# soedinglab/MMseqs2

Hardware: AMD Instinct MI355X
Metric: sw_gcells_per_s (higher is better)
Workload: dtype int16

## Files before the change

mmseqs2_amd/csrc/mmgpu_api.hip:

```cpp
#include <algorithm>
#include <atomic>
#include <thread>
#include <cmath>
#include <cstdio>
#include <cstring>
#include <numeric>
#include <string>
#include <vector>

#include "mmgpu_internal.h"

#include <chrono>

using namespace mmgpu;

namespace mmgpu {
thread_local std::string g_last_error;
}
using mmgpu::g_last_error;

extern "C" const char *mmgpu_last_error(void) { return g_last_error.c_str(); }

extern "C" int mmgpu_init(mmgpu_ctx **out, int device_id) {
    if (!out) return fail(MMGPU_ERR_ARG, "mmgpu_init: ctx is NULL");
// ... 818 lines not shown
        const bool same_list = d > from && Q.target_ids == qs[deferred[d - 1].query].target_ids && Q.n_targets == qs[deferred[d - 1].query].n_targets;
        if (!same_list) {
            ord.resize(Q.n_targets);
            std::iota(ord.begin(), ord.end(), 0u);
            for (uint32_t k = 0; k < Q.n_targets; k++)
                if (Q.target_ids[k] >= tv.n) { P.bad = true; break; }
            if (P.bad) continue;
            std::stable_sort(ord.begin(), ord.end(), [&](uint32_t a, uint32_t bb) {
                return tv.h_len[Q.target_ids[a]] > tv.h_len[Q.target_ids[bb]];
            });
        }
        for (uint32_t k = 0; k < Q.n_targets; k++) {
            const uint32_t t = Q.target_ids[ord[k]];
            hit_target[D.hit_cursor + k] = t;
            hit_out[D.hit_cursor + k] = D.out_cursor + ord[k];
            P.sum_cells += (uint64_t)Q.qlen * tv.h_len[t];
            P.max_tlen = std::max(P.max_tlen, tv.h_len[t]);
        }
        for (uint32_t k = 0; k < Q.n_targets;) {
            uint64_t jc = 0;
            uint32_t e = k;
            while (e < Q.n_targets && e - k < JOB_HITS) {
                const uint32_t stop = std::min<uint32_t>(e + D.round, Q.n_targets);
                for (; e < stop; e++) jc += (uint64_t)Q.qlen * tv.h_len[hit_target[D.hit_cursor + e]];
                const uint32_t held = e - k;
                if (jc >= JOB_CELLS && (held <= 16 || held % JOB_ROUND == 0)) break;
            }
            SwJob j;
            j.query = D.query;
            j.hit_begin = D.hit_cursor + k;
            j.hit_end = D.hit_cursor + e;
            j.shape = D.shape;
            P.jobs.push_back(j);
            P.cells.push_back(jc);
            k = e;
        }
        if (Q.n_targets) P.rev_mid_len = tv.h_len[hit_target[D.hit_cursor + Q.n_targets / 2]];
        if (mode >= MMGPU_SW_START)
            for (uint32_t k = 0; k < Q.n_targets; k++) b->h_out_target[D.out_cursor + k] = Q.target_ids[k];
    }
}

void SwPrepare::cut_list_jobs() {
    per_query.resize(deferred.size());
    static const unsigned host_threads = std::min(16u, std::max(1u, std::thread::hardware_concurrency()));
    const size_t n_thr = std::max<size_t>(1, std::min<size_t>(host_threads, total_hits / 65536 + 1));
    if (n_thr <= 1) {
        cut_list_jobs_of(0, deferred.size());
        return;
    }
    std::vector<std::thread> pool;
    size_t from = 0;
    uint64_t acc = 0;
    const uint64_t share = total_hits / n_thr + 1;
    for (size_t d = 0; d < deferred.size(); d++) {
        acc += qs[deferred[d].query].n_targets;
        if (acc >= share || d + 1 == deferred.size()) {
            pool.emplace_back(&SwPrepare::cut_list_jobs_of, this, from, d + 1);
            from = d + 1;
            acc = 0;
        }
    }
    for (std::thread &t : pool) t.join();
}

int SwPrepare::join_list_jobs() {
    for (size_t d = 0; d < deferred.size(); d++) {
        const Deferred &D = deferred[d];
        PerQuery &P = per_query[d];
        if (P.bad) return fail(MMGPU_ERR_ARG, "mmgpu_sw_prepare: target id out of range");
        b->cells += P.sum_cells;
        max_tlen = std::max(max_tlen, P.max_tlen);
        for (size_t z = 0; z < P.jobs.size(); z++) {
            SwJob j = P.jobs[z];
            if (D.multi) j.shape |= n_multi++ << 8;
            jobs.push_back(j);
            job_cells.push_back(P.cells[z]);
        }
        const uint32_t n_t = qs[D.query].n_targets;
        if (D.multi && mode >= MMGPU_SW_START && n_t)
            add_rev_jobs(D.query, D.hit_cursor, n_t, D.shape, (uint64_t)qs[D.query].qlen * (P.rev_mid_len + 1));
    }
    return MMGPU_OK;
}

void SwPrepare::order_jobs() {
    sorted.resize(jobs.size());
    std::vector<uint32_t> ord(jobs.size());
    std::iota(ord.begin(), ord.end(), 0u);
    std::stable_sort(ord.begin(), ord.end(), [&](uint32_t a, uint32_t bb) {
        const int ga = sw_shape_group(jobs[a].shape & 0xFFu), gb = sw_shape_group(jobs[bb].shape & 0xFFu);
        return ga != gb ? ga < gb : job_cells[a] > job_cells[bb];
    });
    for (size_t z = 0; z < ord.size(); z++) {
        sorted[z] = jobs[ord[z]];
        b->group_begin[sw_shape_group(sorted[z].shape & 0xFFu) + 1]++;
    }
    for (int g = 0; g < SW_GROUPS; g++) b->group_begin[g + 1] += b->group_begin[g];
    b->n_jobs = (uint32_t)sorted.size();
    b->n_multi_jobs = n_multi;
    std::vector<uint32_t> ro(rev_jobs.size());
    std::iota(ro.begin(), ro.end(), 0u);
    std::stable_sort(ro.begin(), ro.end(), [&](uint32_t a, uint32_t bb) { return rev_cells[a] > rev_cells[bb]; });
    for (uint32_t z : ro) sorted.push_back(rev_jobs[z]);
    b->n_rev_jobs = (uint32_t)rev_jobs.size();
}

int SwPrepare::enqueue_uploads() {
    b->pairs = total_hits;
    b->h_qoff = qoff;
    b->from_pf = pf != nullptr;
    b->pf_stride = pf_stride;
    b->slot_stride = pf_stride;
    hipStream_t s = c->stream;
    mat.assign(par->mat, par->mat + par->alphabet * par->alphabet);
    void *pin = nullptr;
    size_t pin_cap = 0, pin_used = 0;
    if (pf) {
        pin_cap = upload_pinned_need(qres.size()) + upload_pinned_need(qcb.size()) + upload_pinned_need(qoff.size() * 4) +
                  upload_pinned_need(qbias.size() * 4) + upload_pinned_need(qminstart.size() * 4) + upload_pinned_need(mat.size()) +
                  upload_pinned_need((jobs.size() + rev_jobs.size()) * sizeof(SwJob)) + upload_pinned_need(qprof.size()) +
                  upload_pinned_need(qprof_off.size() * 4);
        pin = pinned.acquire(c, pin_cap);
    }
    auto up = [&](DevBuf &buf, const auto &vec) { return upload_pinned(buf, vec, s, pin, pin_cap, pin_used); };
    HIP_TRY(up(b->d_qres, qres));
    HIP_TRY(up(b->d_qcb, qcb));
    HIP_TRY(up(b->d_qoff, qoff));
    HIP_TRY(up(b->d_qbias, qbias));
    HIP_TRY(up(b->d_qminstart, qminstart));
    if (b->any_profile) {
        HIP_TRY(up(b->d_qprof, qprof));
        HIP_TRY(up(b->d_qprof_off, qprof_off));
    }
    if (pf) {
        HIP_TRY(b->d_hit_target.alloc(std::max<size_t>((size_t)total_hits, 1) * 4));
        HIP_TRY(b->d_hit_out.alloc(std::max<size_t>((size_t)total_hits, 1) * 4));
        HIP_TRY(b->d_stats.alloc(SW_FROM_PF_STAT_SLOTS * 24));
        HIP_TRY(hipMemsetAsync(b->d_stats.p, 0, SW_FROM_PF_STAT_SLOTS * 24, s));
        HIP_TRY(b->d_pf_counts.alloc(std::max<size_t>(nq, 1) * 4));
        HIP_TRY(b->d_slot_target.alloc(std::max<size_t>((size_t)total_hits, 1) * 4));
    } else {
        HIP_TRY(upload(b->d_hit_target, hit_target, s));
        HIP_TRY(upload(b->d_hit_out, hit_out, s));
    }
    HIP_TRY(up(b->d_mat, mat));
    HIP_TRY(b->d_out.alloc(std::max<size_t>((size_t)total_hits, 1) * sizeof(mmgpu_sw_hit)));
    order_jobs();
    HIP_TRY(up(b->d_jobs, sorted));
    return MMGPU_OK;
}

hipError_t SwPrepare::alloc_scratch(uint32_t longest) {
    b->scratch_cols = longest + 16;
    b->scratch_slots = std::min<uint32_t>(std::max<uint32_t>(std::max<uint32_t>(n_multi, (uint32_t)rev_jobs.size()), 1),
                                          sw_multi_resident_blocks(b->group_lds[SW_GROUPS - 1], mode >= MMGPU_SW_START, c->compute_units));
    hipError_t e = b->d_scratch.alloc((size_t)b->scratch_slots * 4 * 4 * 2 * (size_t)b->scratch_cols * sizeof(uint2));
    if (e != hipSuccess) return e;
    e = b->d_scratch_busy.alloc((size_t)b->scratch_slots * 4);
    if (e != hipSuccess) return e;
    return hipMemsetAsync(b->d_scratch_busy.p, 0, (size_t)b->scratch_slots * 4, c->stream);
}

int SwPrepare::finish_host_lists() {
    if (any_multi) HIP_TRY(alloc_scratch(max_tlen));
    HIP_TRY(hipStreamSynchronize(c->stream));
    return MMGPU_OK;
}

int SwPrepare::order_device_lists() {
    hipStream_t s = c->stream;
    HIP_TRY(hipMemsetAsync(b->d_out.p, 0, std::max<size_t>((size_t)total_hits, 1) * sizeof(mmgpu_sw_hit), s));
    SwFromPfArgs F;
    F.pf_hits = pf->hits;
    F.pf_stride = pf_stride;
    F.hit_count = pf->counts;
    F.stride = pf_stride;
    F.q_off = b->d_qoff.as<uint32_t>();
    F.t_len = tv.len;
    F.hit_target = b->d_hit_target.as<uint32_t>();
    F.hit_out = b->d_hit_out.as<uint32_t>();
    F.cells = b->d_stats.as<unsigned long long>();
    F.pairs = b->d_stats.as<unsigned long long>() + 1;
    F.count_copy = b->d_pf_counts.as<uint32_t>();
    F.slot_target = b->d_slot_target.as<uint32_t>();
    HIP_TRY(launch_sw_from_pf(F, nq, s));
    HIP_TRY(hipStreamSynchronize(s));
    unsigned long long st[3] = {0, 0, 0}, slots[SW_FROM_PF_STAT_SLOTS * 3];
    HIP_TRY(hipMemcpy(slots, b->d_stats.p, sizeof(slots), hipMemcpyDeviceToHost));
    for (int z = 0; z < SW_FROM_PF_STAT_SLOTS; z++) {
        st[0] += slots[z * 3];
        st[1] += slots[z * 3 + 1];
        st[2] = std::max(st[2], slots[z * 3 + 2]);
    }
    b->cells = st[0];
    b->valid_pairs = st[1];
    if (any_multi) {
        HIP_TRY(alloc_scratch((uint32_t)st[2]));
        HIP_TRY(hipStreamSynchronize(s));
    }
    return MMGPU_OK;
}

}

static int sw_prepare_impl(mmgpu_ctx *c, const mmgpu_sw_params *par, const mmgpu_sw_query *qs, uint32_t nq, int mode,
                           const DeviceLists *pf, const mmgpu_sw_masks *masks, mmgpu_sw_batch_t **out) {
    if (!c || !par || !out || (!qs && nq)) return fail(MMGPU_ERR_ARG, "mmgpu_sw_prepare: NULL argument");
    SwPrepare S{c, par, qs, nq, mode, pf, masks};
    if (int e = S.check_params()) return e;
    S.tv = sw_targets(c, nullptr);
    HIP_TRY(hipSetDevice(c->device));
    std::unique_ptr<mmgpu_sw_batch_t, SwBatchFree> b(new mmgpu_sw_batch_t(), SwBatchFree{c});
    S.b = b.get();
    S.new_batch();
    if (int e = S.size_buffers()) return e;
    if (masks)
        if (int e = S.plan_masked()) return e;
    if (int e = S.copy_queries()) return e;
    S.lap("queries copied, buffers sized");
    if (!S.deferred.empty()) {
        S.cut_list_jobs();
        S.lap("lists sorted by target length, jobs cut (threads)");
        if (int e = S.join_list_jobs()) return e;
    }
    S.lap("jobs joined");
    if (int e = S.enqueue_uploads()) return e;
    S.lap("uploads enqueued, jobs ordered");
    if (masks) {
        if (int e = S.gather_masked()) return e;
        S.lap("masked copies of the targets gathered");
    }
    if (int e = pf ? S.order_device_lists() : S.finish_host_lists()) return e;
    S.lap("scratch + stream drained");
    *out = b.release();
    return MMGPU_OK;
}

extern "C" int mmgpu_sw_prepare(mmgpu_ctx *c, const mmgpu_sw_params *par, const mmgpu_sw_query *qs, uint32_t nq,
                                int mode, mmgpu_sw_batch_t **out) {
    return sw_prepare_impl(c, par, qs, nq, mode, nullptr, nullptr, out);
}

extern "C" int mmgpu_sw_prepare_masked(mmgpu_ctx *c, const mmgpu_sw_params *par, const mmgpu_sw_query *qs, uint32_t nq, int mode,
                                       const mmgpu_sw_masks *masks, mmgpu_sw_batch_t **out) {
    if (out) *out = nullptr;
    if (!masks) return fail(MMGPU_ERR_ARG, "mmgpu_sw_prepare_masked: NULL masks");
    return sw_prepare_impl(c, par, qs, nq, mode, nullptr, masks, out);
}

extern "C" int mmgpu_sw_debug_masked_target(mmgpu_ctx *c, mmgpu_sw_batch_t *b, uint32_t pair, uint8_t *out, size_t cap, uint32_t *len) {
    if (!c || !b) return fail(MMGPU_ERR_ARG, "mmgpu_sw_debug_masked_target: NULL argument");
    if (!b->masked) return fail(MMGPU_ERR_STATE, "mmgpu_sw_debug_masked_target: not a batch of mmgpu_sw_prepare_masked");
    if (pair >= b->m_h_len.size()) return fail(MMGPU_ERR_ARG, "mmgpu_sw_debug_masked_target: pair index out of range");
    const uint32_t l = b->m_h_len[pair];
    const size_t bytes = ((size_t)l + 3) & ~(size_t)3;
    if (len) *len = l;
    if (!out && cap == 0) return MMGPU_OK;
    if (cap < bytes || (!out && bytes)) return fail(MMGPU_ERR_ARG, "mmgpu_sw_debug_masked_target: buffer too small (needs (len + 3) & ~3 bytes)");
    HIP_TRY(hipSetDevice(c->device));
    HIP_TRY(hipStreamSynchronize(c->stream));
    uint32_t off4 = 0;
    HIP_TRY(hipMemcpy(&off4, b->m_off4.as<uint32_t>() + pair, 4, hipMemcpyDeviceToHost));
    if (bytes) HIP_TRY(hipMemcpy(out, b->m_res.as<uint8_t>() + (size_t)off4 * 4, bytes, hipMemcpyDeviceToHost));
    return MMGPU_OK;
}

extern "C" int mmgpu_sw_prepare_from_pf(mmgpu_ctx *c, const mmgpu_sw_params *par, const mmgpu_sw_query *qs, uint32_t nq,
                                        int mode, mmgpu_pf_batch_t *pf, mmgpu_sw_batch_t **out) {
    if (!pf) return fail(MMGPU_ERR_ARG, "mmgpu_sw_prepare_from_pf: NULL prefilter batch");
    DeviceLists L;
    uint32_t pf_nq = 0;
    if (!pf_batch_device_lists(pf, &L.hits, &L.counts, &L.stride, &pf_nq))
        return fail(MMGPU_ERR_STATE, "mmgpu_sw_prepare_from_pf: the prefilter batch was never run, or is an exchange batch of a sharded run");
    if (pf_nq != nq) return fail(MMGPU_ERR_ARG, "mmgpu_sw_prepare_from_pf: query count differs from the prefilter batch");
    return sw_prepare_impl(c, par, qs, nq, mode, &L, nullptr, out);
}

extern "C" int mmgpu_sw_prepare_from_lists(mmgpu_ctx *c, const mmgpu_sw_params *par, const mmgpu_sw_query *qs, uint32_t nq, int mode,
                                           const void *d_hits, const void *d_counts, uint32_t stride, mmgpu_sw_batch_t **out) {
    if ((!d_hits || !d_counts) && nq) return fail(MMGPU_ERR_ARG, "mmgpu_sw_prepare_from_lists: NULL list pointers");
    if (stride == 0) return fail(MMGPU_ERR_ARG, "mmgpu_sw_prepare_from_lists: stride must be >= 1");
    DeviceLists L;
    L.hits = (const mmgpu_pf_hit *)d_hits;
    L.counts = (const uint32_t *)d_counts;
    L.stride = stride;
    return sw_prepare_impl(c, par, qs, nq, mode, &L, nullptr, out);
}

extern "C" int mmgpu_sw_prepare_owned(mmgpu_ctx *c, const mmgpu_sw_params *par, const mmgpu_sw_query *qs, uint32_t nq, int mode,
                                      mmgpu_pf_batch_t *merged, mmgpu_sw_batch_t **out) {
    if (!c || !merged || !out) return fail(MMGPU_ERR_ARG, "mmgpu_sw_prepare_owned: NULL argument");
    if (!c->shard.on) return fail(MMGPU_ERR_STATE, "mmgpu_sw_prepare_owned: no shard set (mmgpu_pf_set_shard)");
    const mmgpu_pf_hit *mh = nullptr;
    const uint32_t *mc = nullptr;
    uint32_t stride = 0, mnq = 0;
    if (!mmgpu::pf_batch_merged_lists(merged, &mh, &mc, &stride, &mnq)) return fail(MMGPU_ERR_STATE, "mmgpu_sw_prepare_owned: the prefilter batch holds no merged lists (mmgpu_pf_exchange_merge first)");
    if (mnq != nq) return fail(MMGPU_ERR_ARG, "mmgpu_sw_prepare_owned: query count differs from the prefilter batch");
    HIP_TRY(hipSetDevice(c->device));
    DevBuf lh, lc, ls;
    lh.bind(c->cache); lc.bind(c->cache); ls.bind(c->cache);
    HIP_TRY(lh.alloc(std::max<size_t>((size_t)nq * stride, 1) * sizeof(mmgpu_pf_hit)));
    HIP_TRY(lc.alloc(std::max<size_t>(nq, 1) * 4));
    HIP_TRY(ls.alloc(std::max<size_t>((size_t)nq * stride, 1) * 4));
    PfLocalizeArgs A;
    A.hits = mh;
    A.counts = mc;
// ... 950 lines not shown
```

mmseqs2_amd/csrc/sw_kernel.hip:

```cpp
#include "mmgpu_internal.h"
#include "pf_device.h"

namespace mmgpu {

namespace {

constexpr int GROUP = 16;
constexpr int WAVES = 4;
constexpr int GROUPS_PER_WAVE = 64 / GROUP;
constexpr int HITS_PER_WAVE = 2 * GROUPS_PER_WAVE;
constexpr unsigned NEG2 = 0x80008000u;

typedef short s16x2 __attribute__((ext_vector_type(2)));
typedef unsigned short u16x2 __attribute__((ext_vector_type(2)));

__device__ __forceinline__ unsigned pk_add_sat(unsigned a, unsigned b) {
    return __builtin_bit_cast(unsigned, __builtin_elementwise_add_sat(__builtin_bit_cast(s16x2, a),
                                                                      __builtin_bit_cast(s16x2, b)));
}
__device__ __forceinline__ unsigned pk_max_s(unsigned a, unsigned b) {
    return __builtin_bit_cast(unsigned, __builtin_elementwise_max(__builtin_bit_cast(s16x2, a),
                                                                  __builtin_bit_cast(s16x2, b)));
}
__device__ __forceinline__ unsigned pk_max_u(unsigned a, unsigned b) {
    return __builtin_bit_cast(unsigned, __builtin_elementwise_max(__builtin_bit_cast(u16x2, a),
                                                                  __builtin_bit_cast(u16x2, b)));
}
__device__ __forceinline__ unsigned pk_sub_sat_u(unsigned a, unsigned b) {
    return __builtin_bit_cast(unsigned, __builtin_elementwise_sub_sat(__builtin_bit_cast(u16x2, a),
                                                                      __builtin_bit_cast(u16x2, b)));
}
__device__ __forceinline__ unsigned bfi(unsigned mask, unsigned a, unsigned b) {
    return (a & mask) | (b & ~mask);
}
__device__ __forceinline__ unsigned from_lane_above(unsigned head, unsigned v) {
    return __builtin_amdgcn_update_dpp(head, v, 0x111 , 0xF, 0xF, false);
}

#ifndef MMGPU_SW_PREFETCH
#define MMGPU_SW_PREFETCH 1
#endif
#define SW_KEEP_IN_ROW(x) asm volatile("" : "+v"(x))

template <int R>
struct Tile {
    static constexpr int ROWS = GROUP * R;
    static constexpr int LANE_STRIDE = lane_stride_bytes(R);
    static constexpr int ROW_STRIDE = GROUP * LANE_STRIDE;
};
static_assert(GROUP == 16, "sw_profile_bytes and sw_tiles (mmgpu_internal.h) assume 16-lane groups");

template <int R, bool REV>
__device__ __forceinline__ void build_profile(unsigned char *lds, const uint8_t *q, const int8_t *cb, int qlen,
                                              int tile_base, const int8_t *mat, int alphabet, const int8_t *prof) {
    using T = Tile<R>;
    const int total = (alphabet + 1) * T::ROWS;
    for (int idx = threadIdx.x; idx < total; idx += blockDim.x) {
        const int letter = idx / T::ROWS;
        const int row = idx - letter * T::ROWS;
        const int rg = tile_base + row;
        short v = (short)-32768;
        if (letter < alphabet && rg < qlen) {
            const int qi = REV ? (qlen - 1 - rg) : rg;
            v = prof ? (short)prof[letter * qlen + qi] : (short)((int)mat[letter * alphabet + q[qi]] + (int)cb[qi]);
        }
        const int lane = row / R, r = row - lane * R;
        *reinterpret_cast<short *>(lds + letter * T::ROW_STRIDE + lane * T::LANE_STRIDE + r * 2) = v;
    }
}

__device__ __forceinline__ bool sw_rev_wanted(const SwLaunch &L, uint32_t slot, int min_start) {
    const mmgpu_sw_hit &f = L.out[slot];
    const int s = f.score;
    if (L.rev_mode == 2) return s > 0 && L.rev_force[slot] != 0;
    return s > 0 && s >= min_start && !(L.rev_mode == 1 && f.word != 0);
}

constexpr int SW_REV_JOB_HITS = 1024;
static_assert(SW_REV_JOB_HITS == SW_REV_JOB_MAX, "host and kernel disagree on the reverse job size");
static_assert(SW_LDS_HEADER == SW_REV_JOB_HITS * 2 + 64, "the header holds the live hits and the scheduling words");

template <int R, bool MULTI, bool REV, bool PF>
__device__ __forceinline__ void sw_body(const SwLaunch &L, const SwJob job) {
    using T = Tile<R>;
    extern __shared__ __attribute__((aligned(16))) unsigned char lds_all[];
    uint16_t *live = reinterpret_cast<uint16_t *>(lds_all);
    uint32_t *live_wave = reinterpret_cast<uint32_t *>(lds_all + SW_REV_JOB_HITS * 2);
    uint32_t *next_chunk = reinterpret_cast<uint32_t *>(lds_all + SW_REV_JOB_HITS * 2 + 16);
    unsigned char *lds = lds_all + SW_LDS_HEADER;
    if (MULTI) __builtin_amdgcn_s_setprio(3);
    const int lane = threadIdx.x & 63;
    const int wave = __builtin_amdgcn_readfirstlane(threadIdx.x >> 6);
    const int g = lane & (GROUP - 1);
    const int grp = lane / GROUP;

    const uint32_t qbeg = L.q_off[job.query];
    const int qlen = (int)(L.q_off[job.query + 1] - qbeg);
    const uint8_t *q = L.q_res + qbeg;
    const int8_t *cb = L.q_cb + qbeg;
    const int qbias = L.q_bias[job.query];
    const int8_t *prof = nullptr;
    if (L.q_prof_off) {
        const uint32_t po = L.q_prof_off[job.query];
        if (po != 0xFFFFFFFFu) prof = L.q_prof + po;
    }
    const int n_tiles = MULTI ? (int)sw_tiles((uint32_t)qlen, R) : 1;
    const uint32_t tile_bytes = sw_profile_bytes(R, L.alphabet);
    const bool resident = MULTI && sw_multi_resident((uint32_t)n_tiles, R, L.alphabet, L.resident_lds);
    const bool dynamic = !MULTI || resident;
    auto build_all_tiles = [&]() {
        for (int tile = 0; tile < n_tiles; ++tile)
            build_profile<R, REV>(lds + (uint32_t)tile * tile_bytes, q, cb, qlen, tile * T::ROWS, L.mat, L.alphabet, prof);
        __syncthreads();
    };

    const unsigned go2 = (unsigned)L.gap_open * 0x10001u;
    const unsigned ge2 = (unsigned)L.gap_extend * 0x10001u;
    const unsigned pad_letter = (unsigned)L.alphabet;

    if (threadIdx.x == 0) *next_chunk = 0;
    if (!MULTI && !REV) {
        build_profile<R, REV>(lds, q, cb, qlen, 0, L.mat, L.alphabet, prof);
        __syncthreads();
    }
    if (MULTI && !REV && resident) build_all_tiles();

    uint32_t n_hits = job.hit_end - job.hit_begin;
    if (REV) {
        const int min_start = L.q_minstart[job.query];
        uint32_t total = 0;
        for (uint32_t base = 0; base < n_hits; base += WAVES * 64) {
            const uint32_t idx = base + threadIdx.x;
            bool pass = false;
            if (idx < n_hits) pass = sw_rev_wanted(L, L.hit_out[job.hit_begin + idx], min_start);
            const unsigned long long bal = __ballot(pass);
            if (lane == 0) live_wave[wave] = (uint32_t)__popcll(bal);
            __syncthreads();
            uint32_t before = 0, round_total = 0;
#pragma unroll
            for (int w = 0; w < WAVES; ++w) {
                const uint32_t c = live_wave[w];
                before += w < wave ? c : 0u;
                round_total += c;
            }
            if (pass) live[total + before + (uint32_t)__popcll(bal & ((1ull << lane) - 1ull))] = (uint16_t)idx;
            total += round_total;
            __syncthreads();
        }
        n_hits = total;
        if (n_hits == 0) return;
        if (!MULTI) {
            build_profile<R, REV>(lds, q, cb, qlen, 0, L.mat, L.alphabet, prof);
            __syncthreads();
        }
        if (MULTI && resident) build_all_tiles();
    }
    const uint32_t n_iter = (n_hits + WAVES * HITS_PER_WAVE - 1) / (WAVES * HITS_PER_WAVE);

    for (uint32_t it = 0; dynamic || it < n_iter; ++it) {
        uint32_t chunk = it * WAVES + wave;
        if (dynamic) {
            if (lane == 0) chunk = atomicAdd(next_chunk, 1u);
            chunk = __builtin_amdgcn_readfirstlane(chunk);
        }
        const uint32_t slot0 = chunk * HITS_PER_WAVE;
        if (dynamic && slot0 >= n_hits) break;

        const uint32_t sA = slot0 + grp * 2, sB = sA + 1;
        const bool vA = sA < n_hits, vB = sB < n_hits;
        const uint32_t hA = job.hit_begin + (REV ? (uint32_t)live[vA ? sA : 0] : sA);
        const uint32_t hB = job.hit_begin + (REV ? (uint32_t)live[vB ? sB : 0] : sB);
        const uint32_t tA = vA ? L.hit_target[hA] : 0u, tB = vB ? L.hit_target[hB] : 0u;
        const uint8_t *pA = L.t_res + (size_t)L.t_off4[tA] * 4;
        const uint8_t *pB = L.t_res + (size_t)L.t_off4[tB] * 4;
        int colsA = vA ? (int)L.t_len[tA] : 0, colsB = vB ? (int)L.t_len[tB] : 0;
        int r0A = 0, r0B = 0;
        int endA = 0, endB = 0;
        unsigned rev_target = 0xFFFFFFFFu;
        if (REV) {
            mmgpu_sw_hit fa, fb;
            fa.score = 0; fa.q_end = 0; fa.t_end = 0;
            fb = fa;
            if (vA) fa = L.out[L.hit_out[hA]];
            if (vB) fb = L.out[L.hit_out[hB]];
            colsA = vA ? fa.t_end + 1 : 0;
            colsB = vB ? fb.t_end + 1 : 0;
            endA = colsA > 0 ? fa.t_end : 0;
            endB = colsB > 0 ? fb.t_end : 0;
            r0A = colsA > 0 ? qlen - 1 - fa.q_end : 0;
            r0B = colsB > 0 ? qlen - 1 - fb.q_end : 0;
            rev_target = (colsA > 0 ? (unsigned)fa.score & 0xFFFFu : 0xFFFFu) | ((colsB > 0 ? (unsigned)fb.score & 0xFFFFu : 0xFFFFu) << 16);
        }
        int ncols = colsA > colsB ? colsA : colsB;
        ncols = max(ncols, __shfl_xor(ncols, 16));
        ncols = max(ncols, __shfl_xor(ncols, 32));
        ncols = __builtin_amdgcn_readfirstlane(ncols);
        const int nsteps = ncols + GROUP - 1;

        unsigned long long bestA = 0, bestB = 0;

        uint2 *scr = nullptr;
        if (MULTI) scr = L.scratch + ((size_t)((job.shape >> 8) * WAVES + wave) * GROUPS_PER_WAVE + grp) * 2 * L.scratch_cols;

        for (int tile = 0; tile < n_tiles; ++tile) {
            const int tile_base = tile * T::ROWS;
            if (MULTI && !resident) {
                __syncthreads();
                build_profile<R, REV>(lds, q, cb, qlen, tile_base, L.mat, L.alphabet, prof);
                __syncthreads();
            }
            const unsigned char *const lds_tile = MULTI && resident ? lds + (uint32_t)tile * tile_bytes : lds;
            const uint2 *scr_in = MULTI ? scr + (size_t)((tile + 1) & 1) * L.scratch_cols : nullptr;
            uint2 *scr_out = MULTI ? scr + (size_t)(tile & 1) * L.scratch_cols : nullptr;
            const bool has_above = MULTI && tile > 0;
            const bool has_below = MULTI && tile + 1 < n_tiles;

            unsigned Hp[R], E[R], aux[R];
#pragma unroll
            for (int r = 0; r < R; ++r) { Hp[r] = 0; E[r] = 0; aux[r] = 0; }
            if (REV) {
#pragma unroll
                for (int r = 0; r < R; ++r) {
                    const int rg = tile_base + g * R + r;
                    aux[r] = (rg >= r0A ? 0xFFFFu : 0u) | (rg >= r0B ? 0xFFFF0000u : 0u);
                }
            }
            unsigned vmax = 0, bestcol = 0xFFFFFFFFu;
            unsigned rev_rowA = 0, rev_rowB = 0;
            unsigned Hup_prev = 0;
            unsigned out_H = 0, out_F = 0;

            auto letters4 = [&](const uint8_t *p, int end, int k) -> unsigned {
                if (!REV) return reinterpret_cast<const unsigned *>(p)[k];
                int o = end - 3 - 4 * k;
                o = o < -3 ? -3 : o;
                unsigned w;
                __builtin_memcpy(&w, p + o, 4);
                return w;
            };
            unsigned wA = letters4(pA, endA, 0), wB = letters4(pB, endB, 0);
            unsigned wA_next = letters4(pA, endA, 1), wB_next = letters4(pB, endB, 1);
#ifndef MMGPU_SW_UP_DEPTH
#define MMGPU_SW_UP_DEPTH 4
#endif
            constexpr int UPD = MMGPU_SW_UP_DEPTH;
            uint2 up[UPD];
#pragma unroll
            for (int k = 0; k < UPD; ++k) up[k] = make_uint2(0, 0);
            if (has_above) {
                const int last = ncols - 1 < 0 ? 0 : ncols - 1;
#pragma unroll
                for (int k = 0; k < UPD; ++k) up[k] = scr_in[min(k, last)];
            }

            constexpr int ND = (R + 1) / 2;
            unsigned pav_next[PF ? ND : 1], pbv_next[PF ? ND : 1];
            auto load_rows = [&](unsigned letters, unsigned *pav, unsigned *pbv) {
                const unsigned a = letters & 0xFFu, b = (letters >> 8) & 0xFFu;
                const uint4 *rowA = reinterpret_cast<const uint4 *>(lds_tile + a * T::ROW_STRIDE + g * T::LANE_STRIDE);
                const uint4 *rowB = reinterpret_cast<const uint4 *>(lds_tile + b * T::ROW_STRIDE + g * T::LANE_STRIDE);
#pragma unroll
                for (int k = 0; k < ND / 4; ++k) {
                    const uint4 pa = rowA[k], pb = rowB[k];
                    pav[4 * k] = pa.x; pav[4 * k + 1] = pa.y; pav[4 * k + 2] = pa.z; pav[4 * k + 3] = pa.w;
                    pbv[4 * k] = pb.x; pbv[4 * k + 1] = pb.y; pbv[4 * k + 2] = pb.z; pbv[4 * k + 3] = pb.w;
                }
                if constexpr (ND % 4 >= 2) {
                    const uint2 pa = *reinterpret_cast<const uint2 *>(rowA + ND / 4);
                    const uint2 pb = *reinterpret_cast<const uint2 *>(rowB + ND / 4);
                    pav[(ND / 4) * 4] = pa.x; pav[(ND / 4) * 4 + 1] = pa.y;
                    pbv[(ND / 4) * 4] = pb.x; pbv[(ND / 4) * 4 + 1] = pb.y;
                }
                if constexpr (ND % 2 == 1) {
                    pav[ND - 1] = reinterpret_cast<const unsigned *>(rowA)[ND - 1];
                    pbv[ND - 1] = reinterpret_cast<const unsigned *>(rowB)[ND - 1];
                }
            };
            unsigned let = pad_letter * 0x101u;
            auto head_letters = [&](int c, int j) -> unsigned {
                const unsigned sh = (unsigned)(REV ? 3 - j : j) * 8u;
                const unsigned la0 = __builtin_amdgcn_ubfe(wA, sh, 8u);
                const unsigned lb0 = __builtin_amdgcn_ubfe(wB, sh, 8u);
                return (c < colsA ? la0 : pad_letter) | ((c < colsB ? lb0 : pad_letter) << 8);
            };
            if (PF) {
                let = from_lane_above(head_letters(0, 0), let);
                load_rows(let, pav_next, pbv_next);
            }

            for (int s0 = PF ? -1 : 0; s0 < nsteps; s0 += 4) {
            const int jn = min(4, nsteps - s0);
#pragma nounroll
            for (int j = PF && s0 < 0 ? 1 : 0; j < jn; ++j) {
                const int s = s0 + j;
                unsigned head_let = 0;
                if (!PF) head_let = head_letters(s, j);
                const unsigned Hup = from_lane_above(up[0].x, out_H);
                unsigned f = from_lane_above(up[0].y, out_F);
                if (!PF) let = from_lane_above(head_let, let);
                if (has_above) {
#pragma unroll
                    for (int k = 0; k + 1 < UPD; ++k) up[k] = up[k + 1];
                    int c = s + UPD; if (c > ncols - 1) c = ncols - 1; if (c < 0) c = 0;
                    up[UPD - 1] = scr_in[c];
                }
                unsigned pav[ND], pbv[ND];
                if (PF) {
#pragma unroll
                    for (int k = 0; k < ND; ++k) { pav[k] = pav_next[k]; pbv[k] = pbv_next[k]; }
                } else {
                    load_rows(let, pav, pbv);
                }

                unsigned hd = Hup_prev;
                Hup_prev = Hup;
                unsigned cmax = 0;
                unsigned pre[R], es[R];
#pragma unroll
                for (int r = 0; r < R; ++r) {
                    unsigned P = __builtin_amdgcn_perm(pbv[r / 2], pav[r / 2], (r & 1) ? 0x07060302u : 0x05040100u);
                    if (REV) P = __builtin_amdgcn_bitop3_b32(aux[r], P, NEG2, 0xCA);
                    pre[r] = pk_max_s(pk_add_sat(r == 0 ? hd : Hp[r - 1], P), E[r]);
                    es[r] = pk_sub_sat_u(E[r], ge2);
                }
                if (PF) {
                    let = from_lane_above(head_letters(s + 1, j), let);
                    load_rows(let, pav_next, pbv_next);
                }
#pragma unroll
                for (int r = 0; r < R; ++r) {
                    const unsigned h = pk_max_s(pre[r], f);
                    const unsigned fs = pk_sub_sat_u(f, ge2);
                    const unsigned t = pk_sub_sat_u(h, go2);
                    cmax = pk_max_u(cmax, h);
                    if (MULTI) SW_KEEP_IN_ROW(cmax);
                    f = pk_max_u(fs, t);
                    E[r] = pk_max_u(es[r], t);
                    SW_KEEP_IN_ROW(E[r]);
                    Hp[r] = h;
                }
                out_H = Hp[R - 1];
                out_F = f;

                const int col = s - g;
                if (has_below && g == GROUP - 1 && col >= 0 && col < ncols) scr_out[col] = make_uint2(out_H, out_F);

                const unsigned nm = pk_max_u(vmax, cmax);
                if (nm != vmax) {
                    const unsigned diff = nm ^ vmax;
                    if (!REV) {
                        const unsigned mask = ((diff & 0xFFFFu) ? 0xFFFFu : 0u) | ((diff >> 16) ? 0xFFFF0000u : 0u);
                        bestcol = bfi(mask, ((unsigned)col & 0xFFFFu) * 0x10001u, bestcol);
#pragma unroll
                        for (int r = 0; r < R; ++r) aux[r] = bfi(mask, Hp[r], aux[r]);
                    } else {
                        const unsigned x = nm ^ rev_target;
                        const bool hitA = (diff & 0xFFFFu) && !(x & 0xFFFFu), hitB = (diff >> 16) && !(x >> 16);
                        if (hitA | hitB) {
                            asm volatile("" ::: "memory");
                            unsigned ra = 0, rb = 0;
#pragma unroll
                            for (int r = R - 1; r >= 0; --r) {
                                if ((Hp[r] & 0xFFFFu) == (rev_target & 0xFFFFu)) ra = (unsigned)r;
                                if ((Hp[r] >> 16) == (rev_target >> 16)) rb = (unsigned)r;
                            }
                            if (hitA) { bestcol = (bestcol & 0xFFFF0000u) | ((unsigned)col & 0xFFFFu); rev_rowA = ra; }
                            if (hitB) { bestcol = (bestcol & 0xFFFFu) | ((unsigned)col << 16); rev_rowB = rb; }
                        }
                    }
                    vmax = nm;
                }
            }
            {
                wA = wA_next; wB = wB_next;
                const int k = ((s0 + (PF ? 1 : 0)) >> 2) + 2;
                wA_next = letters4(pA, endA, k); wB_next = letters4(pB, endB, k);
            }
            }

            unsigned rowA_first = rev_rowA, rowB_first = rev_rowB;
            unsigned sA = vmax & 0xFFFFu, sB = vmax >> 16;
            if (!REV) {
#pragma unroll
                for (int r = R - 1; r >= 0; --r) {
                    if ((aux[r] & 0xFFFFu) == sA) rowA_first = (unsigned)r;
                    if ((aux[r] >> 16) == sB) rowB_first = (unsigned)r;
                }
            } else {
                sA = sA == (rev_target & 0xFFFFu) ? sA : 0u;
                sB = sB == (rev_target >> 16) ? sB : 0u;
            }
            const unsigned rgA = (unsigned)(tile_base + g * R) + rowA_first;
            const unsigned rgB = (unsigned)(tile_base + g * R) + rowB_first;
            unsigned long long keyA = sA ? ((unsigned long long)sA << 32) | ((0xFFFFu - (bestcol & 0xFFFFu)) << 16) | (0xFFFFu - rgA) : 0ull;
            unsigned long long keyB = sB ? ((unsigned long long)sB << 32) | ((0xFFFFu - (bestcol >> 16)) << 16) | (0xFFFFu - rgB) : 0ull;
#pragma unroll
            for (int m = 1; m < GROUP; m <<= 1) {
                const unsigned long long oa = __shfl_xor(keyA, m), ob = __shfl_xor(keyB, m);
                keyA = oa > keyA ? oa : keyA;
                keyB = ob > keyB ? ob : keyB;
            }
            bestA = keyA > bestA ? keyA : bestA;
            bestB = keyB > bestB ? keyB : bestB;
        }

        if (g == 0) {
#pragma unroll
            for (int half = 0; half < 2; ++half) {
                const bool valid = half ? vB : vA;
                if (!valid) continue;
                const unsigned long long key = half ? bestB : bestA;
                const uint32_t h = half ? hB : hA;
                const int score = (int)(key >> 32);
                const int col = 0xFFFF - (int)((key >> 16) & 0xFFFFu);
                const int row = 0xFFFF - (int)(key & 0xFFFFu);
                mmgpu_sw_hit *o = L.out + L.hit_out[h];
                if (!REV) {
                    mmgpu_sw_hit res;
                    res.score = score;
                    res.q_end = score ? row : 0;
                    res.t_end = score ? col : -1;
                    res.q_start = -1;
                    res.t_start = -1;
                    res.word = (score + qbias >= 255) ? 1 : 0;
                    *o = res;
                } else {
                    const int end = half ? endB : endA;
                    const int cols = half ? colsB : colsA;
                    if (cols > 0) {
                        o->t_start = (score == o->score) ? end - col : -2;
                        o->q_start = (score == o->score) ? qlen - 1 - row : -2;
                    }
                }
            }
        }
    }
}

template <int R, bool MULTI, bool BOTH>
__device__ __forceinline__ void sw_passes(const SwLaunch &L, const SwJob &job) {
    if constexpr (R <= SW_MAX_R) {
        constexpr bool PF = MMGPU_SW_PREFETCH && !MULTI && (BOTH || R <= 24);
        if (!(BOTH && L.rev_only)) sw_body<R, MULTI, false, PF>(L, job);
        if constexpr (BOTH && !MULTI) {
            __threadfence_block();
            __syncthreads();
            sw_body<R, MULTI, true, PF>(L, job);
        }
    }
}

#ifndef MMGPU_SW_WAVES_G0F
#define MMGPU_SW_WAVES_G0F 4
#endif
#ifndef MMGPU_SW_WAVES_G0B
#define MMGPU_SW_WAVES_G0B 2
#endif
#ifndef MMGPU_SW_WAVES_G1F
#define MMGPU_SW_WAVES_G1F 3
#endif
#ifndef MMGPU_SW_WAVES_G1B
#define MMGPU_SW_WAVES_G1B 2
#endif
#define MMGPU_SW_MULTI_ALL                                                                                                          \
    MMGPU_SW_MULTI(8) MMGPU_SW_MULTI(9) MMGPU_SW_MULTI(10) MMGPU_SW_MULTI(11) MMGPU_SW_MULTI(12) MMGPU_SW_MULTI(13) MMGPU_SW_MULTI(14) \
    MMGPU_SW_MULTI(15) MMGPU_SW_MULTI(16) MMGPU_SW_MULTI(17) MMGPU_SW_MULTI(18) MMGPU_SW_MULTI(19) MMGPU_SW_MULTI(20) MMGPU_SW_MULTI(21) \
    MMGPU_SW_MULTI(22) MMGPU_SW_MULTI(23) MMGPU_SW_MULTI(24) MMGPU_SW_MULTI(25) MMGPU_SW_MULTI(26) MMGPU_SW_MULTI(27) MMGPU_SW_MULTI(28) \
    MMGPU_SW_MULTI(29) MMGPU_SW_MULTI(30) MMGPU_SW_MULTI(31) MMGPU_SW_MULTI(32)
template <int G, bool BOTH>
__global__ __launch_bounds__(WAVES * 64)
__attribute__((amdgpu_waves_per_eu(G == 0 ? (BOTH ? MMGPU_SW_WAVES_G0B : MMGPU_SW_WAVES_G0F)
                                           : (G == 1 ? (BOTH ? MMGPU_SW_WAVES_G1B : MMGPU_SW_WAVES_G1F) : SW_MIN_WAVES),
                                   G == 1 && BOTH ? MMGPU_SW_WAVES_G1B : 8))) void sw_kernel(SwLaunch L) {
    SwJob job = L.jobs[blockIdx.x];
    if (L.q_hit_count) {
        const uint32_t lim = job.query * L.hit_stride + L.q_hit_count[job.query];
        job.hit_end = job.hit_end < lim ? job.hit_end : lim;
        if (job.hit_end <= job.hit_begin) return;
    }
    __shared__ uint32_t scratch_slot;
    const bool claims = G == SW_GROUPS - 1 && (job.shape & 0xFFu) >= 32u;
    if (claims) {
        if (threadIdx.x == 0) {
            uint32_t s = blockIdx.x % L.scratch_slots;
            while (atomicCAS(&L.scratch_busy[s], 0u, 1u) != 0u) s = s + 1 == L.scratch_slots ? 0u : s + 1;
            scratch_slot = s;
        }
        __syncthreads();
        job.shape = (job.shape & 0xFFu) | (scratch_slot << 8);
    }
#define MMGPU_SW_SINGLE(R) case (R) - 1: sw_passes<R, false, BOTH>(L, job); break;
#define MMGPU_SW_MULTI(R) case 32 + (R) - 1: sw_passes<R, true, BOTH>(L, job); break;
    if constexpr (G == 0) {
        switch (job.shape & 0xFFu) {
            MMGPU_SW_SINGLE(1) MMGPU_SW_SINGLE(2) MMGPU_SW_SINGLE(3) MMGPU_SW_SINGLE(4) MMGPU_SW_SINGLE(5) MMGPU_SW_SINGLE(6)
            MMGPU_SW_SINGLE(7) MMGPU_SW_SINGLE(8) MMGPU_SW_SINGLE(9) MMGPU_SW_SINGLE(10) MMGPU_SW_SINGLE(11) MMGPU_SW_SINGLE(12)
            default: break;
        }
    } else if constexpr (G == 1) {
        switch (job.shape & 0xFFu) {
            MMGPU_SW_SINGLE(13) MMGPU_SW_SINGLE(14) MMGPU_SW_SINGLE(15) MMGPU_SW_SINGLE(16) MMGPU_SW_SINGLE(17) MMGPU_SW_SINGLE(18)
            MMGPU_SW_SINGLE(19) MMGPU_SW_SINGLE(20) MMGPU_SW_SINGLE(21) MMGPU_SW_SINGLE(22) MMGPU_SW_SINGLE(23) MMGPU_SW_SINGLE(24)
            default: break;
        }
    } else if constexpr (SW_GROUPS == 4 && G == 2) {
        switch (job.shape & 0xFFu) {
            MMGPU_SW_SINGLE(25) MMGPU_SW_SINGLE(26) MMGPU_SW_SINGLE(27) MMGPU_SW_SINGLE(28) MMGPU_SW_SINGLE(29) MMGPU_SW_SINGLE(30)
            MMGPU_SW_SINGLE(31) MMGPU_SW_SINGLE(32)
            default: break;
        }
    } else if constexpr (SW_GROUPS == 4) {
        switch (job.shape & 0xFFu) {
            MMGPU_SW_MULTI_ALL
            default: break;
        }
    } else {
        switch (job.shape & 0xFFu) {
            MMGPU_SW_SINGLE(25) MMGPU_SW_SINGLE(26) MMGPU_SW_SINGLE(27) MMGPU_SW_SINGLE(28) MMGPU_SW_SINGLE(29) MMGPU_SW_SINGLE(30)
            MMGPU_SW_SINGLE(31) MMGPU_SW_SINGLE(32)
            MMGPU_SW_MULTI_ALL
            default: break;
        }
    }
#undef MMGPU_SW_SINGLE
#undef MMGPU_SW_MULTI
#undef MMGPU_SW_MULTI_ALL
    if (claims) {
        __syncthreads();
        if (threadIdx.x == 0) {
            __threadfence();
            atomicExch(&L.scratch_busy[scratch_slot], 0u);
// ... 156 lines not shown
```

Baseline: 4507.

## Batch inter-tile boundary loads per 16 columns and precompute packed letter blocks

Replaces the per-step sliding window of scratch boundary loads with one coalesced load of 16 boundary cells per group. Each lane holds one cell and the values are rotated across lanes with DPP, so the load runs every 16 steps instead of every step. Boundary stores are shifted so the last-row output is written one step later, plus a final store after the loop. Letter extraction is moved to a per-4-column block that packs both targets' letters with perm into a 64-bit queue, padding only near the shorter target's end. Non-multi tiles use a bound-ctrl zero DPP instead of a boundary value. The risks are more complex indexing, extra registers, and the scratch column padding needed for the aligned reads.

```diff
diff --git a/mmseqs2_amd/csrc/mmgpu_api.hip b/mmseqs2_amd/csrc/mmgpu_api.hip
--- a/mmseqs2_amd/csrc/mmgpu_api.hip
+++ b/mmseqs2_amd/csrc/mmgpu_api.hip
@@ -994,7 +994,7 @@
 }
 
 hipError_t SwPrepare::alloc_scratch(uint32_t longest) {
-    b->scratch_cols = longest + 16;
+    b->scratch_cols = ((longest + 15u) & ~15u) + 16;
     b->scratch_slots = std::min<uint32_t>(std::max<uint32_t>(std::max<uint32_t>(n_multi, (uint32_t)rev_jobs.size()), 1),
                                           sw_multi_resident_blocks(b->group_lds[SW_GROUPS - 1], mode >= MMGPU_SW_START, c->compute_units));
     hipError_t e = b->d_scratch.alloc((size_t)b->scratch_slots * 4 * 4 * 2 * (size_t)b->scratch_cols * sizeof(uint2));
diff --git a/mmseqs2_amd/csrc/sw_kernel.hip b/mmseqs2_amd/csrc/sw_kernel.hip
--- a/mmseqs2_amd/csrc/sw_kernel.hip
+++ b/mmseqs2_amd/csrc/sw_kernel.hip
@@ -35,6 +35,9 @@
 }
 __device__ __forceinline__ unsigned from_lane_above(unsigned head, unsigned v) {
     return __builtin_amdgcn_update_dpp(head, v, 0x111 , 0xF, 0xF, false);
+}
+__device__ __forceinline__ unsigned from_lane_above_or_zero(unsigned v) {
+    return __builtin_amdgcn_update_dpp(0u, v, 0x111 , 0xF, 0xF, true);
 }
 
 #ifndef MMGPU_SW_PREFETCH
@@ -196,11 +199,19 @@
         ncols = max(ncols, __shfl_xor(ncols, 32));
         ncols = __builtin_amdgcn_readfirstlane(ncols);
         const int nsteps = ncols + GROUP - 1;
+        int mincols = colsA < colsB ? colsA : colsB;
+        mincols = min(mincols, __shfl_xor(mincols, 16));
+        mincols = min(mincols, __shfl_xor(mincols, 32));
+        mincols = __builtin_amdgcn_readfirstlane(mincols);
 
         unsigned long long bestA = 0, bestB = 0;
 
         uint2 *scr = nullptr;
-        if (MULTI) scr = L.scratch + ((size_t)((job.shape >> 8) * WAVES + wave) * GROUPS_PER_WAVE + grp) * 2 * L.scratch_cols;
+        unsigned scr_grp = 0;
+        if (MULTI) {
+            scr = L.scratch + (size_t)((job.shape >> 8) * WAVES + wave) * GROUPS_PER_WAVE * 2 * L.scratch_cols;
+            scr_grp = (unsigned)grp * 2u * L.scratch_cols;
+        }
 
         for (int tile = 0; tile < n_tiles; ++tile) {
             const int tile_base = tile * T::ROWS;
@@ -240,17 +251,14 @@
             };
             unsigned wA = letters4(pA, endA, 0), wB = letters4(pB, endB, 0);
             unsigned wA_next = letters4(pA, endA, 1), wB_next = letters4(pB, endB, 1);
-#ifndef MMGPU_SW_UP_DEPTH
-#define MMGPU_SW_UP_DEPTH 4
-#endif
-            constexpr int UPD = MMGPU_SW_UP_DEPTH;
-            uint2 up[UPD];
-#pragma unroll
-            for (int k = 0; k < UPD; ++k) up[k] = make_uint2(0, 0);
+            uint2 bnd = make_uint2(0, 0), bnd_next = make_uint2(0, 0);
+            auto boundary16 = [&](int m) -> uint2 {
+                const int last = ncols - 1 < 0 ? 0 : ncols - 1;
+                return scr_in[scr_grp + (unsigned)min(16 * m + g - (m > 0 ? 1 : 0), last)];
+            };
             if (has_above) {
-                const int last = ncols - 1 < 0 ? 0 : ncols - 1;
-#pragma unroll
-                for (int k = 0; k < UPD; ++k) up[k] = scr_in[min(k, last)];
+                bnd = boundary16(0);
+                bnd_next = boundary16(1);
             }
 
             constexpr int ND = (R + 1) / 2;
@@ -277,32 +285,53 @@
                 }
             };
             unsigned let = pad_letter * 0x101u;
+            constexpr bool LETTER_BLOCKS = MULTI || REV || R >= 7;
+            constexpr bool LETTER_QUEUE = !MULTI && R < 7;
+            unsigned long long lq = 0;
+            auto letter_block = [&](int k) {
+                if (!LETTER_BLOCKS) return;
+                unsigned a = wA, b = wB;
+                if (4 * k + 4 > mincols) {
+                    const unsigned pad4 = pad_letter * 0x01010101u;
+                    const int na = min(max(colsA - 4 * k, 0), 4), nb = min(max(colsB - 4 * k, 0), 4);
+                    const unsigned ma = REV ? ~(unsigned)(0xFFFFFFFFull >> (8 * na)) : (unsigned)((1ull << (8 * na)) - 1ull);
+                    const unsigned mb = REV ? ~(unsigned)(0xFFFFFFFFull >> (8 * nb)) : (unsigned)((1ull << (8 * nb)) - 1ull);
+                    a = bfi(ma, a, pad4);
+                    b = bfi(mb, b, pad4);
+                }
+                const unsigned lo = __builtin_amdgcn_perm(b, a, REV ? 0x06020703u : 0x05010400u);
+                const unsigned hi = __builtin_amdgcn_perm(b, a, REV ? 0x04000501u : 0x07030602u);
+                lq = ((unsigned long long)hi << 32) | lo;
+            };
             auto head_letters = [&](int c, int j) -> unsigned {
+                if (LETTER_BLOCKS && LETTER_QUEUE) { const unsigned v = (unsigned)lq; lq >>= 16; return v; }
+                if (LETTER_BLOCKS) return (unsigned)(lq >> (16 * j));
                 const unsigned sh = (unsigned)(REV ? 3 - j : j) * 8u;
                 const unsigned la0 = __builtin_amdgcn_ubfe(wA, sh, 8u);
                 const unsigned lb0 = __builtin_amdgcn_ubfe(wB, sh, 8u);
                 return (c < colsA ? la0 : pad_letter) | ((c < colsB ? lb0 : pad_letter) << 8);
             };
-            if (PF) {
-                let = from_lane_above(head_letters(0, 0), let);
-                load_rows(let, pav_next, pbv_next);
-            }
-
-            for (int s0 = PF ? -1 : 0; s0 < nsteps; s0 += 4) {
+            letter_block(0);
+            let = from_lane_above(head_letters(0, 0), let);
+            if (PF) load_rows(let, pav_next, pbv_next);
+
+            for (int s0 = -1; s0 < nsteps; s0 += 4) {
+            if (MULTI && s0 > 0 && ((s0 + 1) & 15) == 0) {
+                bnd = bnd_next;
+                if (has_above) bnd_next = boundary16(((s0 + 1) >> 4) + 1);
+            }
             const int jn = min(4, nsteps - s0);
 #pragma nounroll
-            for (int j = PF && s0 < 0 ? 1 : 0; j < jn; ++j) {
+            for (int j = s0 < 0 ? 1 : 0; j < jn; ++j) {
                 const int s = s0 + j;
-                unsigned head_let = 0;
-                if (!PF) head_let = head_letters(s, j);
-                const unsigned Hup = from_lane_above(up[0].x, out_H);
-                unsigned f = from_lane_above(up[0].y, out_F);
-                if (!PF) let = from_lane_above(head_let, let);
-                if (has_above) {
-#pragma unroll
-                    for (int k = 0; k + 1 < UPD; ++k) up[k] = up[k + 1];
-                    int c = s + UPD; if (c > ncols - 1) c = ncols - 1; if (c < 0) c = 0;
-                    up[UPD - 1] = scr_in[c];
+                if (has_below && s >= GROUP) {
+                    if (g == GROUP - 1) (scr_out + (s - GROUP))[scr_grp] = make_uint2(out_H, out_F);
+                }
+                const unsigned Hup = MULTI ? from_lane_above(bnd.x, out_H) : from_lane_above_or_zero(out_H);
+                unsigned f = MULTI ? from_lane_above(bnd.y, out_F) : from_lane_above_or_zero(out_F);
+                if (MULTI) {
+                    bnd.x = __builtin_amdgcn_update_dpp(bnd.x, bnd.x, 0x12F, 0xF, 0xF, false);
+                    bnd.y = __builtin_amdgcn_update_dpp(bnd.y, bnd.y, 0x12F, 0xF, 0xF, false);
                 }
                 unsigned pav[ND], pbv[ND];
                 if (PF) {
@@ -323,17 +352,14 @@
                     pre[r] = pk_max_s(pk_add_sat(r == 0 ? hd : Hp[r - 1], P), E[r]);
                     es[r] = pk_sub_sat_u(E[r], ge2);
                 }
-                if (PF) {
-                    let = from_lane_above(head_letters(s + 1, j), let);
-                    load_rows(let, pav_next, pbv_next);
-                }
+                let = from_lane_above(head_letters(s + 1, j), let);
+                if (PF) load_rows(let, pav_next, pbv_next);
 #pragma unroll
                 for (int r = 0; r < R; ++r) {
                     const unsigned h = pk_max_s(pre[r], f);
                     const unsigned fs = pk_sub_sat_u(f, ge2);
                     const unsigned t = pk_sub_sat_u(h, go2);
                     cmax = pk_max_u(cmax, h);
-                    if (MULTI) SW_KEEP_IN_ROW(cmax);
                     f = pk_max_u(fs, t);
                     E[r] = pk_max_u(es[r], t);
                     SW_KEEP_IN_ROW(E[r]);
@@ -343,7 +369,6 @@
                 out_F = f;
 
                 const int col = s - g;
-                if (has_below && g == GROUP - 1 && col >= 0 && col < ncols) scr_out[col] = make_uint2(out_H, out_F);
 
                 const unsigned nm = pk_max_u(vmax, cmax);
                 if (nm != vmax) {
@@ -373,10 +398,12 @@
             }
             {
                 wA = wA_next; wB = wB_next;
-                const int k = ((s0 + (PF ? 1 : 0)) >> 2) + 2;
+                const int k = ((s0 + 1) >> 2) + 2;
                 wA_next = letters4(pA, endA, k); wB_next = letters4(pB, endB, k);
-            }
-            }
+                letter_block(k - 1);
+            }
+            }
+            if (has_below && ncols > 0 && g == GROUP - 1) (scr_out + (ncols - 1))[scr_grp] = make_uint2(out_H, out_F);
 
             unsigned rowA_first = rev_rowA, rowB_first = rev_rowB;
             unsigned sA = vmax & 0xFFFFu, sB = vmax >> 16;
```

After: 4665, median of 6. 3.5% higher.
